# arkflow-rs/arkflow

Measured on AMD Instinct MI355X. Metric: rows/sec, higher is better.
Workload: dtype bf16; 1 GPU; model=generate→sql(filter)→mlp_anomaly[16→256→256→1], global_batch=8192, seq_len=1, parallelism=dp1, batch_size_per_gpu=8192, workers=1, filter=WHERE f0 >= 0.2

## Files before the change

### arkflow_amd/csrc/bindings.cpp

```cpp
#include <hip/hip_runtime.h>
#include <torch/extension.h>
#include <ATen/hip/HIPContext.h>

#include <algorithm>
#include <cstdint>
#include <limits>
#include <tuple>
#include <vector>

#include "gemm_api.h"
#include "kernels_api.h"
#include "relational_api.h"

namespace {

hipStream_t cur_stream() {
  return at::hip::getCurrentHIPStream().stream();
}

void check_cuda(const torch::Tensor& t, const char* name) {
  TORCH_CHECK(t.is_cuda(), name, " must be on GPU");
  TORCH_CHECK(t.is_contiguous(), name, " must be contiguous");
}

// ... 141 lines not shown
  TORCH_CHECK(keys.scalar_type() == torch::kInt64, "keys must be int64");
  int64_t n = keys.numel();
  auto opts32 = keys.options().dtype(torch::kInt32);
  if (n == 0)
    return {torch::empty({0}, opts32), torch::empty({0}, keys.options())};
  uint32_t tsize = next_pow2((uint32_t)std::max<int64_t>(n * 2, 64));
  auto table_keys = torch::empty({(int64_t)tsize}, keys.options());
  auto table_gids = torch::empty({(int64_t)tsize}, opts32);
  auto counter = torch::zeros({1}, opts32);
  auto gids = torch::empty({n}, opts32);
  auto st = cur_stream();
  launch_hash_build(keys.data_ptr<int64_t>(), n,
                    table_keys.data_ptr<int64_t>(),
                    table_gids.data_ptr<int32_t>(), tsize,
                    counter.data_ptr<int32_t>(), gids.data_ptr<int32_t>(), st);
  int64_t g = counter.item<int32_t>();
  auto uniq = torch::empty({g}, keys.options());
  launch_hash_export(table_keys.data_ptr<int64_t>(),
                     table_gids.data_ptr<int32_t>(), tsize,
                     uniq.data_ptr<int64_t>(), st);
  return {gids, uniq};
}

torch::Tensor segment_reduce_f32(torch::Tensor vals, torch::Tensor gids,
                                 int64_t g, int64_t op) {
  check_cuda(vals, "vals");
  check_cuda(gids, "gids");
  TORCH_CHECK(vals.scalar_type() == torch::kFloat32, "vals must be f32");
  auto g32 = gids.scalar_type() == torch::kInt32 ? gids
                                                 : gids.to(torch::kInt32);
  auto out = torch::zeros({g}, vals.options());
  if (vals.numel() == 0) return out;
  torch::Tensor scratch;
  int32_t* scratch_ptr = nullptr;
  if (op != 0) {
    scratch = torch::empty({g}, vals.options().dtype(torch::kInt32));
    scratch_ptr = scratch.data_ptr<int32_t>();
  }
  launch_segment_reduce_f32(vals.data_ptr<float>(), g32.data_ptr<int32_t>(),
                            vals.numel(), (int)g, (int)op,
                            out.data_ptr<float>(), scratch_ptr, cur_stream());
  return out;
}

std::tuple<torch::Tensor, torch::Tensor> join_inner_i64(torch::Tensor lk,
                                                        torch::Tensor rk) {
  check_cuda(lk, "left_keys");
  check_cuda(rk, "right_keys");
  TORCH_CHECK(lk.scalar_type() == torch::kInt64 &&
                  rk.scalar_type() == torch::kInt64,
              "join keys must be int64");
  int64_t nl = lk.numel(), nr = rk.numel();
  auto opts64 = lk.options();
  auto opts32 = lk.options().dtype(torch::kInt32);
  if (nl == 0 || nr == 0)
    return {torch::empty({0}, opts64), torch::empty({0}, opts64)};
  uint32_t tsize = next_pow2((uint32_t)std::max<int64_t>(nr * 2, 64));
  auto table_keys = torch::empty({(int64_t)tsize}, opts64);
  auto table_head = torch::empty({(int64_t)tsize}, opts32);
  auto next = torch::empty({nr}, opts32);
  auto st = cur_stream();
  launch_join_build(rk.data_ptr<int64_t>(), nr, table_keys.data_ptr<int64_t>(),
                    table_head.data_ptr<int32_t>(), next.data_ptr<int32_t>(),
                    tsize, st);
  auto counts = torch::empty({nl}, opts32);
  launch_join_probe_count(lk.data_ptr<int64_t>(), nl,
                          table_keys.data_ptr<int64_t>(),
                          table_head.data_ptr<int32_t>(),
                          next.data_ptr<int32_t>(), rk.data_ptr<int64_t>(),
                          tsize, counts.data_ptr<int32_t>(), st);
  auto [offs, total_t] = exscan(counts);
  int64_t total = total_t.item<int32_t>();
  auto l_out = torch::empty({total}, opts64);
  auto r_out = torch::empty({total}, opts64);
  if (total)
    launch_join_probe_emit(lk.data_ptr<int64_t>(), nl,
                           table_keys.data_ptr<int64_t>(),
                           table_head.data_ptr<int32_t>(),
                           next.data_ptr<int32_t>(), rk.data_ptr<int64_t>(),
                           tsize, offs.data_ptr<int32_t>(),
                           l_out.data_ptr<int64_t>(),
                           r_out.data_ptr<int64_t>(), st);
  return {l_out, r_out};
}

torch::Tensor device_vec_f32(const c10::optional<torch::Tensor>& v,
                             int64_t numel, const char* name) {
  if (!v.has_value() || !v->defined()) return torch::Tensor();
  TORCH_CHECK(v->is_cuda(), name, " must be on GPU");
  TORCH_CHECK(v->numel() == numel, name, " must have ", numel, " elements");
  return v->scalar_type() == torch::kFloat32
             ? v->contiguous()
             : v->to(torch::kFloat32).contiguous();
}

torch::Tensor check_gemm_args(const torch::Tensor& A, const torch::Tensor& Bt,
                              const c10::optional<torch::Tensor>& bias) {
  check_cuda(A, "A");
  check_cuda(Bt, "Bt");
  TORCH_CHECK(A.scalar_type() == torch::kBFloat16 &&
                  Bt.scalar_type() == torch::kBFloat16,
              "gemm_bf16 requires bf16 inputs");
  TORCH_CHECK(A.dim() == 2 && Bt.dim() == 2, "A [M,K], Bt [N,K]");
  int64_t K = A.size(1);
  TORCH_CHECK(Bt.size(1) == K, "K mismatch");
  TORCH_CHECK(K % 32 == 0 && K >= 32, "K must be a multiple of 32");
  return device_vec_f32(bias, Bt.size(0), "bias");
}

GemmArgs gemm_args(const torch::Tensor& A, const torch::Tensor& Bt,
                   const torch::Tensor& bias_f, torch::Tensor& C,
                   int64_t act) {
  return GemmArgs{A.data_ptr(), Bt.data_ptr(),
                  bias_f.defined() ? bias_f.data_ptr<float>() : nullptr,
                  C.data_ptr(), (int)A.size(0), (int)Bt.size(0),
                  (int)A.size(1), (int)act, cur_stream()};
}

torch::Tensor gemm_bf16(torch::Tensor A, torch::Tensor Bt,
                        c10::optional<torch::Tensor> bias, int64_t act) {
  auto bias_f = check_gemm_args(A, Bt, bias);
  int64_t M = A.size(0), K = A.size(1), N = Bt.size(0);
  auto C = torch::empty({M, N}, A.options());
  if (M == 0 || N == 0) return C;
  GemmArgs g = gemm_args(A, Bt, bias_f, C, act);
  int64_t t256 = ((M + 255) / 256) * ((N + 255) / 256);
  int rc = (t256 >= 128 && K >= 1536 && N >= 2048)
               ? launch_gemm_bf16(GEMM_8P256S, &g)
               : GEMM_BAD_SHAPE;
  if (rc != GEMM_OK) {
    int64_t t128grid = ((M + 127) / 128) * ((N + 127) / 128);
    if (t128grid < 208) {
      rc = launch_gemm_bf16(GEMM_SKINNY, &g);
    } else {
      rc = (K % 64 == 0) ? launch_gemm_bf16(GEMM_K64S, &g) : GEMM_BAD_SHAPE;
      if (rc != GEMM_OK) rc = launch_gemm_bf16(GEMM_BK32, &g);
    }
  }
  TORCH_CHECK(rc == GEMM_OK, "gemm_bf16: no kernel for this shape");
  return C;
}

torch::Tensor gemv_bf16_f32(torch::Tensor x, torch::Tensor w, double bias) {
  check_cuda(x, "x");
  check_cuda(w, "w");
  TORCH_CHECK(x.scalar_type() == torch::kBFloat16 &&
              w.scalar_type() == torch::kBFloat16, "bf16 required");
  TORCH_CHECK(x.dim() == 2 && w.numel() == x.size(1), "x [M,K], w [K]");
  auto out = torch::empty({x.size(0)}, x.options().dtype(torch::kFloat32));
  if (x.size(0) == 0) return out;
  launch_gemv_bf16_f32(x.data_ptr(), w.data_ptr(), (float)bias, x.size(0),
                       (int)x.size(1), out.data_ptr<float>(), cur_stream());
  return out;
}

void gen_fields(torch::Tensor block, c10::optional<torch::Tensor> key,
                std::vector<double> lo, std::vector<double> width,
                int64_t key_lo, int64_t key_range, torch::Tensor ctr) {
  check_cuda(block, "block");
  TORCH_CHECK(block.dim() == 2 && block.scalar_type() == torch::kFloat32,
              "block must be [nf, n] f32");
  TORCH_CHECK(ctr.scalar_type() == torch::kInt64 && ctr.numel() == 2,
              "ctr must be int64[2] on device");
  int nf = (int)block.size(0);
  int64_t n = block.size(1);
  TORCH_CHECK((int)lo.size() == nf && (int)width.size() == nf);
  std::vector<float> lof(nf), wf(nf);
  for (int f = 0; f < nf; ++f) { lof[f] = (float)lo[f]; wf[f] = (float)width[f]; }
  int64_t* key_ptr = nullptr;
  if (key.has_value() && key->defined()) {
    check_cuda(*key, "key");
    TORCH_CHECK(key->numel() == n && key->scalar_type() == torch::kInt64);
    key_ptr = key->data_ptr<int64_t>();
  } else {
    key_range = 0;
  }
  launch_gen_fields(block.data_ptr<float>(), key_ptr, n, lof.data(),
                    wf.data(), nf, key_lo, key_range,
                    (unsigned long long*)ctr.data_ptr<int64_t>(),
                    cur_stream());
}

void genfiltpack(std::vector<double> lo, std::vector<double> width,
                 int64_t key_lo, int64_t key_range, int64_t n, int64_t fidx,
                 int64_t op, double scalar,
                 std::vector<torch::Tensor> outs,
                 c10::optional<torch::Tensor> key_out,
                 c10::optional<torch::Tensor> feats,
                 torch::Tensor count_out, torch::Tensor counts_ws,
                 torch::Tensor bar, torch::Tensor ctr) {
  int nf = (int)outs.size();
  TORCH_CHECK(nf >= 1 && nf <= 32, "1..32 float columns");
  TORCH_CHECK((int)lo.size() == nf && (int)width.size() == nf);
  TORCH_CHECK(fidx >= 0 && fidx < nf, "fidx out of range");
  TORCH_CHECK(count_out.scalar_type() == torch::kInt32 &&
              count_out.numel() == 1);
  TORCH_CHECK(counts_ws.scalar_type() == torch::kInt32 &&
              counts_ws.numel() >= (n + 1023) / 1024);
  TORCH_CHECK(bar.scalar_type() == torch::kInt64 && bar.numel() >= 1);
  TORCH_CHECK(ctr.scalar_type() == torch::kInt64 && ctr.numel() == 2);
  std::vector<float> lof(nf), wf(nf);
  std::vector<float*> optr(nf);
  for (int f = 0; f < nf; ++f) {
    lof[f] = (float)lo[f];
    wf[f] = (float)width[f];
    check_cuda(outs[f], "out col");
    TORCH_CHECK(outs[f].numel() >= n &&
                outs[f].scalar_type() == torch::kFloat32);
    optr[f] = outs[f].data_ptr<float>();
  }
  int64_t* kptr = nullptr;
  if (key_out.has_value() && key_out->defined()) {
    TORCH_CHECK(key_out->numel() >= n &&
                key_out->scalar_type() == torch::kInt64);
    kptr = key_out->data_ptr<int64_t>();
  } else {
    key_range = 0;
  }
  void* fptr = nullptr;
  int dpad = 0;
  if (feats.has_value() && feats->defined()) {
    TORCH_CHECK(feats->dim() == 2 &&
                feats->scalar_type() == torch::kBFloat16 &&
                feats->size(0) >= n && feats->size(1) >= nf);
    fptr = feats->data_ptr();
    dpad = (int)feats->size(1);
  }
  int rc = launch_genfiltpack(
      lof.data(), wf.data(), nf, key_lo, key_range, n, (int)fidx, (int)op,
      (float)scalar, optr.data(), kptr, fptr, dpad,
      count_out.data_ptr<int32_t>(), counts_ws.data_ptr<int32_t>(),
      (unsigned long long*)bar.data_ptr<int64_t>(),
      (unsigned long long*)ctr.data_ptr<int64_t>(), cur_stream());
  TORCH_CHECK(rc == 0, "genfiltpack: batch too large for the in-kernel "
              "barrier (max 256K rows) — use the multi-kernel chain");
}

void featpack(std::vector<torch::Tensor> srcs, torch::Tensor out) {
  TORCH_CHECK(!srcs.empty() && srcs.size() <= 32, "1..32 feature columns");
  check_cuda(out, "out");
  TORCH_CHECK(out.dim() == 2 && out.scalar_type() == torch::kBFloat16,
              "out must be [n, kpad] bf16");
  int64_t n = out.size(0);
  int kpad = (int)out.size(1);
  TORCH_CHECK((int64_t)srcs.size() <= out.size(1),
              "out has fewer columns than sources");
  if (n == 0) return;
  bool f64 = srcs[0].scalar_type() == torch::kFloat64;
  if (f64) {
    std::vector<const double*> ptrs;
    for (auto& s : srcs) {
      check_cuda(s, "src");
      TORCH_CHECK(s.numel() >= n && s.scalar_type() == torch::kFloat64);
      ptrs.push_back(s.data_ptr<double>());
    }
    launch_featpack64(ptrs.data(), (int)ptrs.size(), kpad, n,
                      out.data_ptr(), cur_stream());
    return;
  }
  std::vector<const float*> ptrs;
  for (auto& s : srcs) {
    check_cuda(s, "src");
    TORCH_CHECK(s.numel() >= n && s.scalar_type() == torch::kFloat32);
    ptrs.push_back(s.data_ptr<float>());
  }
  launch_featpack(ptrs.data(), (int)ptrs.size(), kpad, n, out.data_ptr(),
                  cur_stream());
}

torch::Tensor gemm_bf16_variant(torch::Tensor A, torch::Tensor Bt,
                                c10::optional<torch::Tensor> bias,
                                int64_t act, int64_t variant) {
  auto bias_f = check_gemm_args(A, Bt, bias);
  auto C = torch::empty({A.size(0), Bt.size(0)}, A.options());
  if (C.numel() == 0) return C;
  GemmArgs g = gemm_args(A, Bt, bias_f, C, act);
  int rc = variant == (int)variant ? launch_gemm_bf16((int)variant, &g)
                                   : (int)GEMM_BAD_VARIANT;
  TORCH_CHECK(rc != GEMM_BAD_VARIANT, "unknown gemm variant ", variant);
  TORCH_CHECK(rc == GEMM_OK, "K = ", g.K,
              " not supported by gemm variant ", variant);
  return C;
}

torch::Tensor layernorm_bf16(torch::Tensor x, torch::Tensor gamma,
                             torch::Tensor beta, double eps,
                             c10::optional<torch::Tensor> residual) {
  check_cuda(x, "x");
  TORCH_CHECK(x.scalar_type() == torch::kBFloat16, "x must be bf16");
  TORCH_CHECK(x.dim() >= 1 && x.size(-1) > 0, "x must be [..., n], n > 0");
  int64_t n = x.size(-1);
  TORCH_CHECK(n % 8 == 0, "inner dim must be a multiple of 8");
  int64_t rows = x.numel() / n;
  TORCH_CHECK(gamma.defined() && beta.defined(), "gamma and beta required");
  auto g = device_vec_f32(gamma, n, "gamma");
  auto b = device_vec_f32(beta, n, "beta");
  auto out = torch::empty_like(x);
  const void* res_ptr = nullptr;
  if (residual.has_value() && residual->defined()) {
    check_cuda(*residual, "residual");
    TORCH_CHECK(residual->scalar_type() == torch::kBFloat16,
                "residual must be bf16");
    TORCH_CHECK(residual->sizes() == x.sizes(),
                "residual must have x's shape");
    res_ptr = residual->data_ptr();
  }
// ... 591 lines not shown
void check_rows(const torch::Tensor& t, const char* name,
                torch::ScalarType ty, int64_t n) {
  check_cuda(t, name);
  TORCH_CHECK(t.scalar_type() == ty, name, " has the wrong dtype");
  TORCH_CHECK(t.dim() == 1 && t.numel() == n, name, " must have one entry ",
              "per row");
}

torch::Tensor segmented_scan(torch::Tensor vals, torch::Tensor head,
                             int64_t op, bool reverse) {
  int64_t n = vals.numel();
  TORCH_CHECK(n < (int64_t(1) << 31), "row indices are int32");
  TORCH_CHECK(op >= SCAN_SUM && op <= SCAN_MAX, "unknown scan op ", op);
  check_rows(vals, "values", torch::kFloat64, n);
  check_rows(head, "head", torch::kUInt8, n);
  return seg_scan(vals, head, (int)op, reverse);
}

std::tuple<torch::Tensor, torch::Tensor> window_frame(
    torch::Tensor vals, c10::optional<torch::Tensor> valid,
    torch::Tensor part, c10::optional<int64_t> lo, c10::optional<int64_t> hi,
    int64_t func, c10::optional<torch::Tensor> perm) {
  int64_t n = part.numel();
  TORCH_CHECK(n < (int64_t(1) << 31), "row indices are int32");
  TORCH_CHECK(func >= WF_SUM && func <= WF_COUNT_STAR,
              "unknown window function ", func);
  TORCH_CHECK(!lo || !hi || *lo <= *hi, "frame start is after frame end");
  check_rows(part, "partition ids", torch::kInt64, n);
  check_rows(vals, "values", torch::kFloat64, n);
  if (valid) check_rows(*valid, "validity", torch::kUInt8, n);
  if (perm) check_rows(*perm, "perm", torch::kInt64, n);
  auto f64 = vals.options();
  auto u8 = vals.options().dtype(torch::kUInt8);
  auto out = torch::empty({n}, f64);
  auto out_valid = torch::empty({n}, u8);
  if (n == 0) return {out, out_valid};
  auto st = cur_stream();
  if (lo) lo = std::max(-n, std::min(n, *lo));
  if (hi) hi = std::max(-n, std::min(n, *hi));

  auto head = torch::empty({n}, u8), tail = torch::empty({n}, u8);
  auto head_idx = torch::empty({n}, f64), tail_idx = torch::empty({n}, f64);
  launch_win_bounds(part.data_ptr<int64_t>(), n, head.data_ptr<uint8_t>(),
                    tail.data_ptr<uint8_t>(), head_idx.data_ptr<double>(),
                    tail_idx.data_ptr<double>(), st);
  auto start = seg_scan(head_idx, head, SCAN_MAX, false);
  auto end = seg_scan(tail_idx, tail, SCAN_MIN, true);

  const bool is_sum = func == WF_SUM || func == WF_AVG;
  const bool is_minmax = func == WF_MIN || func == WF_MAX;
  const bool sliding = is_minmax && lo && hi;
  const bool need_count = valid && (is_sum || is_minmax || func == WF_COUNT);
  const int64_t width = sliding ? *hi - *lo + 1 : 1;
  const double inf = std::numeric_limits<double>::infinity();
  const double fill = func == WF_MIN ? inf : func == WF_MAX ? -inf : 0.0;

  torch::Tensor masked, ones, chunk_head, chunk_tail, prefix, suffix, count;
  if (is_sum || is_minmax) masked = torch::empty({n}, f64);
  if (need_count) ones = torch::empty({n}, f64);
  if (sliding) {
    chunk_head = torch::empty({n}, u8);
    chunk_tail = torch::empty({n}, u8);
  }
  auto ptr_f64 = [](const torch::Tensor& t) {
    return t.defined() ? t.data_ptr<double>() : nullptr;
  };
  auto ptr_u8 = [](const torch::Tensor& t) {
    return t.defined() ? t.data_ptr<uint8_t>() : nullptr;
  };
  const uint8_t* valid_p = valid ? valid->data_ptr<uint8_t>() : nullptr;
  if (masked.defined() || ones.defined())
    launch_win_inputs(vals.data_ptr<double>(), valid_p,
                      start.data_ptr<double>(), end.data_ptr<double>(), n,
                      fill, width, ptr_f64(masked), ptr_f64(ones),
                      ptr_u8(chunk_head), ptr_u8(chunk_tail), st);
  if (need_count) count = seg_scan(ones, head, SCAN_SUM, false);
  if (is_sum) prefix = seg_scan(masked, head, SCAN_SUM, false);
  if (is_minmax) {
    const int op = func == WF_MIN ? SCAN_MIN : SCAN_MAX;
    if (sliding || !lo)
      prefix = seg_scan(masked, sliding ? chunk_head : head, op, false);
    if (sliding || lo)
      suffix = seg_scan(masked, sliding ? chunk_tail : tail, op, true);
  }

  FrameArgs a{};
  a.start = start.data_ptr<double>();
  a.end = end.data_ptr<double>();
  a.vals = vals.data_ptr<double>();
  a.valid = valid_p;
  a.prefix = ptr_f64(prefix);
  a.suffix = ptr_f64(suffix);
  a.count = ptr_f64(count);
  a.perm = perm ? perm->data_ptr<int64_t>() : nullptr;
  a.lo = lo.value_or(0);
  a.hi = hi.value_or(0);
  a.lo_unbounded = !lo;
  a.hi_unbounded = !hi;
  a.func = (int)func;
  a.n = n;
  a.out = out.data_ptr<double>();
  a.out_valid = out_valid.data_ptr<uint8_t>();
  launch_win_frame(&a, st);
  return {out, out_valid};
}

}

PYBIND11_MODULE(TORCH_EXTENSION_NAME, m) {
  m.doc() = "arkflow_amd gfx950 native kernels";
  m.def("exclusive_offsets", &exclusive_offsets);
  m.def("take_binary", &take_binary);
  m.def("bytes_match", &bytes_match);
  m.def("attention_qkv_bf16", &attention_qkv_bf16, py::arg("qkv"),
        py::arg("scale"), py::arg("pad") = 8, py::arg("lens") = py::none());
  m.def("mask_to_indices", &mask_to_indices);
  m.def("filter_cmp_scalar", &filter_cmp_scalar);
  m.def("gather", &gather);
  m.def("hash_group_i64", &hash_group_i64);
  m.def("segment_reduce_f32", &segment_reduce_f32);
  m.def("join_inner_i64", &join_inner_i64);
  m.def("gemm_bf16", &gemm_bf16, py::arg("A"), py::arg("Bt"),
        py::arg("bias") = py::none(), py::arg("act") = 0);
  m.def("layernorm_bf16", &layernorm_bf16, py::arg("x"), py::arg("gamma"),
        py::arg("beta"), py::arg("eps") = 1e-5,
        py::arg("residual") = py::none());
  m.def("softmax_bf16", &softmax_bf16, py::arg("x"), py::arg("scale") = 1.0);
  m.def("mapped_int32", &mapped_int32, py::arg("n"));
  m.def("bias_act_bf16", &bias_act_bf16, py::arg("x"),
        py::arg("bias") = py::none(), py::arg("act") = 0);
  m.def("attention_bf16", &attention_bf16, py::arg("q"), py::arg("k"),
        py::arg("v"), py::arg("scale"), py::arg("lens") = py::none());
  m.def("proto_decode", &proto_decode, py::arg("data"),
        py::arg("offsets"), py::arg("fno"), py::arg("kind"),
        py::arg("is_float"), py::arg("slot"), py::arg("n_int"),
        py::arg("n_float"), py::arg("n_str"), py::arg("capture") = false);
  m.def("gather_columns", &gather_columns);
  m.def("gemm_bf16_variant", &gemm_bf16_variant);
  m.def("bytes_hash", &bytes_hash);
  m.def("json_decode", &json_decode);
  m.def("fused_filter_gather", &fused_filter_gather);
  m.def("genfiltpack", &genfiltpack, py::arg("lo"), py::arg("width"),
        py::arg("key_lo"), py::arg("key_range"), py::arg("n"),
        py::arg("fidx"), py::arg("op"), py::arg("scalar"), py::arg("outs"),
        py::arg("key_out"), py::arg("feats"), py::arg("count_out"),
        py::arg("counts_ws"), py::arg("bar"), py::arg("ctr"));
  m.def("fused_filter_agg", &fused_filter_agg);
  m.def("hash_agg_capture", &hash_agg_capture, py::arg("keys"),
        py::arg("nrow"), py::arg("vals"), py::arg("ops"),
        py::arg("table_size"), py::arg("g_cap"),
        py::arg("gcount_out") = c10::nullopt);
  m.def("filter_gather_capture", &filter_gather_capture);
  m.def("gemv_bf16_f32", &gemv_bf16_f32);
  m.def("gen_fields", &gen_fields);
  m.def("featpack", &featpack);
  m.def("radix_argsort", &radix_argsort, py::arg("keys"), py::arg("descending") = false);
  m.def("segmented_scan", &segmented_scan, py::arg("values"), py::arg("head"),
        py::arg("op"), py::arg("reverse") = false);
  m.def("seg_scan_tile_rows", &seg_scan_tile_rows);
  m.def("window_frame", &window_frame, py::arg("values"), py::arg("valid"),
        py::arg("part"), py::arg("lo"), py::arg("hi"), py::arg("func"),
        py::arg("perm") = py::none());
}
```

### arkflow_amd/csrc/gemm_api.h

```cpp
#pragma once
#include <hip/hip_runtime.h>

enum GemmVariant {
  GEMM_BK32 = 0,
  GEMM_8P256 = 1,
  GEMM_8P256S = 2,
  GEMM_2P = 3,
  GEMM_8P128 = 4,
  GEMM_8P128S = 5,
  GEMM_SKINNY = 6,
  GEMM_K64 = 7,
  GEMM_K64S = 8,
  GEMM_K64D = 9,
  GEMM_K64P = 10,
  GEMM_K64W = 11,
  GEMM_K64S3 = 12,
};

enum GemmStatus {
  GEMM_OK = 0,
  GEMM_BAD_SHAPE = 1,
  GEMM_BAD_VARIANT = 2,
};

struct GemmArgs {
  const void* A;
  const void* Bt;
  const float* bias;
  void* C;
  int M, N, K;
  int act;
  hipStream_t stream;
};

extern "C" int launch_gemm_bf16(int variant, const GemmArgs* args);
```

### arkflow_amd/csrc/gemm_common.h

```cpp
#pragma once
#include <hip/hip_runtime.h>

#include <type_traits>

#include "common.h"
#include "gemm_api.h"

typedef __attribute__((ext_vector_type(8))) __bf16 bf16x8;
typedef __attribute__((ext_vector_type(4))) float f32x4;
typedef __attribute__((ext_vector_type(4))) uint32_t u32x4;

enum Act { ACT_NONE = 0, ACT_RELU = 1, ACT_GELU = 2, ACT_SILU = 3 };

DEV_INLINE float apply_act(float x, int act) {
  switch (act) {
    case ACT_RELU: return fmaxf(x, 0.f);
    case ACT_GELU: {
      float c = 0.7978845608028654f * (x + 0.044715f * x * x * x);
      c = fminf(fmaxf(c, -10.f), 10.f);
      float e = __expf(2.f * c);
      return 0.5f * x * (1.f + (e - 1.f) / (e + 1.f));
    }
    case ACT_SILU: return x / (1.f + __expf(-x));
    default: return x;
  }
}

DEV_INLINE int xcd_block_id() {
  int nwg = gridDim.x;
  int bid = blockIdx.x;
  if (nwg >= 16) {
    int q = nwg / 8, r = nwg % 8;
    int xcd = bid % 8, off = bid / 8;
    bid = (xcd < r ? xcd * (q + 1) : r * (q + 1) + (xcd - r) * q) + off;
  }
  return bid;
}


template <int TILE, int BKT, int THREADS>
DEV_INLINE void stage_direct(const __bf16* __restrict__ A,
                             const __bf16* __restrict__ Bt, int row0, int col0,
                             int M, int N, int K, int k0, __bf16* Asm,
                             __bf16* Bsm) {
  constexpr int ROW_BYTES = BKT * 2;
  constexpr int STEPS = TILE * ROW_BYTES / (THREADS * 16);
  const int lane = threadIdx.x & 63;
  const int wid = threadIdx.x >> 6;
#pragma unroll
  for (int it = 0; it < STEPS; ++it) {
    int wbase = wid * 1024 + it * THREADS * 16;
    int lin = wbase + lane * 16;
    int trow = lin / ROW_BYTES;
    int tcol = lin % ROW_BYTES;
    int ga_row = min(row0 + trow, M - 1);
    const char* a_src = (const char*)(A + (int64_t)ga_row * K + k0) + tcol;
    __builtin_amdgcn_global_load_lds(
        (const __attribute__((address_space(1))) uint32_t*)a_src,
        (__attribute__((address_space(3))) uint32_t*)((char*)Asm + wbase),
        16, 0, 0);
    int gb_row = min(col0 + trow, N - 1);
    const char* b_src = (const char*)(Bt + (int64_t)gb_row * K + k0) + tcol;
    __builtin_amdgcn_global_load_lds(
        (const __attribute__((address_space(1))) uint32_t*)b_src,
        (__attribute__((address_space(3))) uint32_t*)((char*)Bsm + wbase),
        16, 0, 0);
  }
}

constexpr int SWZ_BK = 64;
constexpr int SWZ_STEPS = 4;

template <int TILE>
DEV_INLINE void swz_load(const __bf16* __restrict__ A,
                         const __bf16* __restrict__ Bt, int row0, int col0,
                         int M, int N, int K, int k0, u32x4 (&va)[SWZ_STEPS],
                         u32x4 (&vb)[SWZ_STEPS]) {
  const int lin0 = (threadIdx.x >> 6) * 1024 + (threadIdx.x & 63) * 16;
#pragma unroll
  for (int it = 0; it < SWZ_STEPS; ++it) {
    int lin = lin0 + it * (2 * TILE * 16);
    int trow = lin >> 7;
    int tcol = lin & 127;
    int ga_row = min(row0 + trow, M - 1);
    va[it] = *(const u32x4*)((const char*)(A + (int64_t)ga_row * K + k0) +
                             tcol);
    int gb_row = min(col0 + trow, N - 1);
    vb[it] = *(const u32x4*)((const char*)(Bt + (int64_t)gb_row * K + k0) +
                             tcol);
  }
}

template <int TILE>
DEV_INLINE void swz_write(__bf16* Asm, __bf16* Bsm,
                          const u32x4 (&va)[SWZ_STEPS],
                          const u32x4 (&vb)[SWZ_STEPS]) {
  const int lin0 = (threadIdx.x >> 6) * 1024 + (threadIdx.x & 63) * 16;
#pragma unroll
  for (int it = 0; it < SWZ_STEPS; ++it) {
    int lin = lin0 + it * (2 * TILE * 16);
    int trow = lin >> 7;
    int tcol = lin & 127;
    int dst = (trow << 7) + (((tcol >> 4) ^ (trow & 7)) << 4);
    *(u32x4*)((char*)Asm + dst) = va[it];
    *(u32x4*)((char*)Bsm + dst) = vb[it];
  }
}

template <int FM, int FN, int BKT, bool SWZ>
DEV_INLINE void load_frags(const __bf16* Asm, const __bf16* Bsm, int wm,
                           int wn, int ks, bf16x8 (&a_frag)[FM],
                           bf16x8 (&b_frag)[FN]) {
  const int lane = threadIdx.x & 63;
  const int fr = lane & 15;
  const int chunk = ks * 4 + (lane >> 4);
#pragma unroll
  for (int m = 0; m < FM; ++m) {
    int row = wm + m * 16 + fr;
    a_frag[m] =
        *(const bf16x8*)&Asm[row * BKT + (SWZ ? chunk ^ (row & 7) : chunk) * 8];
  }
#pragma unroll
  for (int n = 0; n < FN; ++n) {
    int row = wn + n * 16 + fr;
    b_frag[n] =
        *(const bf16x8*)&Bsm[row * BKT + (SWZ ? chunk ^ (row & 7) : chunk) * 8];
  }
}

template <int FM, int FN>
DEV_INLINE void mma_frags(const bf16x8 (&a_frag)[FM],
                          const bf16x8 (&b_frag)[FN], f32x4 (&acc)[FM][FN]) {
#pragma unroll
  for (int m = 0; m < FM; ++m)
#pragma unroll
    for (int n = 0; n < FN; ++n)
      acc[m][n] = __builtin_amdgcn_mfma_f32_16x16x32_bf16(
          a_frag[m], b_frag[n], acc[m][n], 0, 0, 0);
}

template <int FM, int FN, int BKT, bool SWZ>
DEV_INLINE void mma_slice(const __bf16* Asm, const __bf16* Bsm, int wm, int wn,
                          f32x4 (&acc)[FM][FN]) {
#pragma unroll
  for (int ks = 0; ks < BKT / 32; ++ks) {
    bf16x8 a_frag[FM], b_frag[FN];
    load_frags<FM, FN, BKT, SWZ>(Asm, Bsm, wm, wn, ks, a_frag, b_frag);
    mma_frags<FM, FN>(a_frag, b_frag, acc);
  }
}

template <int ACT, bool HAS_BIAS, int FM, int FN, class RowOf, class ColOf>
DEV_INLINE void store_frags(const f32x4 (&acc)[FM][FN],
                            const float* __restrict__ bias,
                            __bf16* __restrict__ C, int M, int N,
                            RowOf frag_row, ColOf frag_col) {
  const int lane = threadIdx.x & 63;
#pragma unroll
  for (int m = 0; m < FM; ++m) {
#pragma unroll
    for (int n = 0; n < FN; ++n) {
      int col = frag_col(n) + (lane & 15);
      if (col >= N) continue;
      float b = HAS_BIAS ? bias[col] : 0.f;
#pragma unroll
      for (int r = 0; r < 4; ++r) {
        int row = frag_row(m) + (lane >> 4) * 4 + r;
        if (row >= M) continue;
        C[(int64_t)row * N + col] = (__bf16)apply_act(acc[m][n][r] + b, ACT);
      }
    }
  }
}

template <int ACT, bool HAS_BIAS, int FM, int FN>
DEV_INLINE void store_tile(const f32x4 (&acc)[FM][FN],
                           const float* __restrict__ bias,
                           __bf16* __restrict__ C, int M, int N, int wrow,
                           int wcol) {
  store_frags<ACT, HAS_BIAS>(
      acc, bias, C, M, N, [&](int m) { return wrow + m * 16; },
      [&](int n) { return wcol + n * 16; });
}

template <class F>
static void dispatch_epilogue(int act, bool has_bias, F&& f) {
  auto with_act = [&](auto a) {
    if (has_bias) f(a, std::true_type{});
    else f(a, std::false_type{});
  };
  switch (act) {
    case ACT_RELU: with_act(std::integral_constant<int, ACT_RELU>{}); break;
    case ACT_GELU: with_act(std::integral_constant<int, ACT_GELU>{}); break;
    case ACT_SILU: with_act(std::integral_constant<int, ACT_SILU>{}); break;
    default: with_act(std::integral_constant<int, ACT_NONE>{}); break;
  }
}

template <int BMT, int BNT, class Kernel>
static void launch_tiles(Kernel kernel, int threads, size_t lds_bytes,
                         const GemmArgs& g) {
  int tiles_n = cdiv(g.N, BNT);
  hipLaunchKernelGGL(kernel, dim3(cdiv(g.M, BMT) * tiles_n), dim3(threads),
                     lds_bytes, g.stream, (const __bf16*)g.A,
                     (const __bf16*)g.Bt, g.bias, (__bf16*)g.C, g.M, g.N, g.K,
                     tiles_n);
}

int launch_gemm_bf16_8p(const GemmArgs& g, int bm, bool swz);
```

### arkflow_amd/csrc/stepfused.hip

```cpp
#include "common.h"
#include "kernels_api.h"

DEV_INLINE float u01(uint64_t h) {
  return (float)(h >> 40) * (1.0f / 16777216.0f);
}

struct GenSpec {
  float lo[32];
  float width[32];
  int nf;
  int64_t key_lo;
  int64_t key_range;
};

__global__ void gen_fields_kernel(float* __restrict__ block,
                                  int64_t* __restrict__ key, int64_t n,
                                  GenSpec spec,
                                  unsigned long long* __restrict__ ctr) {
  uint64_t c = ctr[0];
  int64_t i = (int64_t)blockIdx.x * blockDim.x + threadIdx.x;
  int64_t stride = (int64_t)gridDim.x * blockDim.x;
  for (; i < n; i += stride) {
    uint64_t base = (c << 32) ^ (uint64_t)i;
#pragma unroll 4
    for (int f = 0; f < spec.nf; ++f) {
      uint64_t h = mix64(base + ((uint64_t)(f + 1) << 52));
      block[(int64_t)f * n + i] = spec.lo[f] + spec.width[f] * u01(h);
    }
    if (spec.key_range > 0) {
      uint64_t h = mix64(base + (0x9E37ull << 48));
      key[i] = spec.key_lo + (int64_t)(h % (uint64_t)spec.key_range);
    }
  }
  __syncthreads();
  if (threadIdx.x == 0) {
    unsigned long long t = atomicAdd(&ctr[1], 1ull);
    if (t == (unsigned long long)gridDim.x - 1) {
      ctr[1] = 0ull;
      ctr[0] = c + 1ull;
      __threadfence();
    }
  }
}

extern "C" void launch_gen_fields(float* block, int64_t* key, int64_t n,
                                  const float* lo, const float* width,
                                  int nf, int64_t key_lo, int64_t key_range,
                                  unsigned long long* ctr, hipStream_t st) {
  GenSpec spec{};
  spec.nf = nf > 32 ? 32 : nf;
  for (int f = 0; f < spec.nf; ++f) {
    spec.lo[f] = lo[f];
    spec.width[f] = width[f];
  }
  spec.key_lo = key_lo;
  spec.key_range = key_range;
  int grid = (int)((n + 255) / 256);
  if (grid > 1024) grid = 1024;
  if (grid < 1) return;
  gen_fields_kernel<<<grid, 256, 0, st>>>(block, key, n, spec, ctr);
}

__global__ void scan_counts_kernel(const int32_t* __restrict__ counts, int nb,
                                   int32_t* __restrict__ offs,
                                   int32_t* __restrict__ total) {
  __shared__ int32_t lds[1024];
  int tid = threadIdx.x;
  int v = tid < nb ? counts[tid] : 0;
  lds[tid] = v;
  __syncthreads();
  for (int s = 1; s < 1024; s <<= 1) {
    int add = tid >= s ? lds[tid - s] : 0;
    __syncthreads();
    lds[tid] += add;
    __syncthreads();
  }
  if (tid < nb) offs[tid] = lds[tid] - v;
  if (tid == nb - 1) *total = lds[tid];
}

extern "C" void launch_scan_counts(const int32_t* counts, int nb,
                                   int32_t* offs, int32_t* total,
                                   hipStream_t st) {
  scan_counts_kernel<<<1, 1024, 0, st>>>(counts, nb, offs, total);
}

struct GfpOuts {
  float* outs[32];
  int64_t* key_out;
  __bf16* feats;
  int32_t* count_out;
  int32_t* counts_ws;
  unsigned long long* bar;
  unsigned long long* ctr;
};

#define GFP_CH 1024

__global__ __launch_bounds__(256)
void genfiltpack_kernel(GenSpec spec, int64_t n, int ch, int fidx, int op,
                        float scalar, int dpad, GfpOuts o) {
  const uint64_t c = o.ctr[0];
  const int b = blockIdx.x, grid = gridDim.x;
  const int tid = threadIdx.x;
  const int lane = tid & 63, wid = tid >> 6;
  const int64_t start = (int64_t)b * ch;
  __shared__ uint16_t loc[GFP_CH];
  __shared__ int wave_base[5];
  __shared__ int lcount_sh;
  __shared__ int base_sh;
  if (tid == 0) lcount_sh = 0;
  __syncthreads();
  for (int s = 0; s < ch / 256; ++s) {
    int64_t idx = start + s * 256 + tid;
    bool pred = false;
    if (idx < n) {
      uint64_t rb = (c << 32) ^ (uint64_t)idx;
      uint64_t h = mix64(rb + ((uint64_t)(fidx + 1) << 52));
      float v = spec.lo[fidx] + spec.width[fidx] * u01(h);
      switch (op) {
        case 0: pred = v < scalar; break;
        case 1: pred = v <= scalar; break;
        case 2: pred = v > scalar; break;
        case 3: pred = v >= scalar; break;
        case 4: pred = v == scalar; break;
        default: pred = v != scalar; break;
      }
    }
    uint64_t ballot = __ballot(pred);
    int rank = __popcll(ballot & lanemask_lt());
    if (lane == 0) wave_base[wid + 1] = __popcll(ballot);
    __syncthreads();
    if (tid == 0) {
      wave_base[0] = lcount_sh;
      for (int w = 1; w <= 4; ++w) wave_base[w] += wave_base[w - 1];
      lcount_sh = wave_base[4];
    }
    __syncthreads();
    if (pred) loc[wave_base[wid] + rank] = (uint16_t)(s * 256 + tid);
    __syncthreads();
  }
  const int lcount = lcount_sh;
  if (tid == 0)
    __hip_atomic_store(&o.counts_ws[b], lcount, __ATOMIC_RELEASE,
                       __HIP_MEMORY_SCOPE_AGENT);
  if (tid == 0) {
    unsigned long long old = atomicAdd(o.bar, 1ull);
    unsigned long long target =
        (old / grid + 1) * (unsigned long long)grid;
    while (__hip_atomic_load(o.bar, __ATOMIC_ACQUIRE,
                             __HIP_MEMORY_SCOPE_AGENT) < target)
      __builtin_amdgcn_s_sleep(8);
  }
  __syncthreads();
  if (tid == 0) {
    int basev = 0, total = 0;
    for (int j = 0; j < grid; ++j) {
      int v = __hip_atomic_load(&o.counts_ws[j], __ATOMIC_RELAXED,
                                __HIP_MEMORY_SCOPE_AGENT);
      if (j < b) basev += v;
      total += v;
    }
    base_sh = basev;
    if (b == 0) *o.count_out = total;
  }
  __syncthreads();
  const int base_out = base_sh;
  for (int j = tid; j < lcount; j += 256) {
    int64_t r = start + loc[j];
    int64_t dst = base_out + j;
    uint64_t rb = (c << 32) ^ (uint64_t)r;
    for (int f = 0; f < spec.nf; ++f) {
      uint64_t h = mix64(rb + ((uint64_t)(f + 1) << 52));
      float v = spec.lo[f] + spec.width[f] * u01(h);
      o.outs[f][dst] = v;
      if (o.feats) o.feats[dst * dpad + f] = (__bf16)v;
    }
    if (spec.key_range > 0) {
      uint64_t h = mix64(rb + (0x9E37ull << 48));
      o.key_out[dst] =
          spec.key_lo + (int64_t)(h % (uint64_t)spec.key_range);
    }
  }
  __syncthreads();
  if (tid == 0) {
    unsigned long long t = atomicAdd(&o.ctr[1], 1ull);
    if (t == (unsigned long long)grid - 1) {
      o.ctr[1] = 0ull;
      o.ctr[0] = c + 1ull;
      __threadfence();
    }
  }
}

extern "C" int launch_genfiltpack(const float* lo, const float* width,
                                  int nf, int64_t key_lo, int64_t key_range,
                                  int64_t n, int fidx, int op, float scalar,
                                  float* const* outs, int64_t* key_out,
                                  void* feats, int dpad, int32_t* count_out,
                                  int32_t* counts_ws,
                                  unsigned long long* bar,
                                  unsigned long long* ctr, hipStream_t st) {
  int ch = GFP_CH;
  while (ch > 256 && (n + ch - 1) / ch < 64) ch >>= 1;
  int grid = (int)((n + ch - 1) / ch);
  if (grid < 1 || grid > 256 || nf > 32) return -1;
  GenSpec spec{};
  spec.nf = nf;
  for (int f = 0; f < nf; ++f) {
    spec.lo[f] = lo[f];
    spec.width[f] = width[f];
  }
  spec.key_lo = key_lo;
  spec.key_range = key_range;
  GfpOuts o{};
  for (int f = 0; f < nf; ++f) o.outs[f] = outs[f];
  o.key_out = key_out;
  o.feats = (__bf16*)feats;
  o.count_out = count_out;
  o.counts_ws = counts_ws;
  o.bar = bar;
  o.ctr = ctr;
  genfiltpack_kernel<<<grid, 256, 0, st>>>(spec, n, ch, fidx, op, scalar,
                                           dpad, o);
  return 0;
}

struct PackSpec {
  const float* src[32];
  int nf;
  int kpad;
};

__global__ void featpack_kernel(PackSpec spec, int64_t n,
                                __bf16* __restrict__ out) {
  int64_t i = (int64_t)blockIdx.x * blockDim.x + threadIdx.x;
  int64_t stride = (int64_t)gridDim.x * blockDim.x;
  for (; i < n; i += stride) {
    __bf16* row = out + i * spec.kpad;
#pragma unroll 4
    for (int f = 0; f < spec.nf; ++f) row[f] = (__bf16)spec.src[f][i];
    for (int f = spec.nf; f < spec.kpad; ++f) row[f] = (__bf16)0.f;
  }
}

extern "C" void launch_featpack(const float** src, int nf, int kpad,
                                int64_t n, void* out, hipStream_t st) {
  PackSpec spec{};
  spec.nf = nf > 32 ? 32 : nf;
  spec.kpad = kpad;
  for (int f = 0; f < spec.nf; ++f) spec.src[f] = src[f];
  int grid = (int)((n + 255) / 256);
  if (grid > 2048) grid = 2048;
  if (grid < 1) return;
  featpack_kernel<<<grid, 256, 0, st>>>(spec, n, (__bf16*)out);
}

struct PackSpec64 {
  const double* src[32];
  int nf;
  int kpad;
};

__global__ void featpack64_kernel(PackSpec64 spec, int64_t n,
                                  __bf16* __restrict__ out) {
  int64_t i = (int64_t)blockIdx.x * blockDim.x + threadIdx.x;
  int64_t stride = (int64_t)gridDim.x * blockDim.x;
  for (; i < n; i += stride) {
    __bf16* row = out + i * spec.kpad;
#pragma unroll 4
    for (int f = 0; f < spec.nf; ++f) {
      float v = (float)spec.src[f][i];
      asm volatile("" : "+v"(v));
      row[f] = (__bf16)v;
    }
    for (int f = spec.nf; f < spec.kpad; ++f) row[f] = (__bf16)0.f;
  }
}

extern "C" void launch_featpack64(const double** src, int nf, int kpad,
                                  int64_t n, void* out, hipStream_t st) {
  PackSpec64 spec{};
  spec.nf = nf > 32 ? 32 : nf;
  spec.kpad = kpad;
  for (int f = 0; f < spec.nf; ++f) spec.src[f] = src[f];
  int grid = (int)((n + 255) / 256);
  if (grid > 2048) grid = 2048;
  if (grid < 1) return;
  featpack64_kernel<<<grid, 256, 0, st>>>(spec, n, (__bf16*)out);
}

__global__ void gemv_bf16_f32_kernel(const __bf16* __restrict__ x,
                                     const __bf16* __restrict__ w,
                                     float bias, int64_t M, int K,
                                     float* __restrict__ out) {
  int64_t wave = ((int64_t)blockIdx.x * blockDim.x + threadIdx.x) >> 6;
  int lane = threadIdx.x & 63;
  int64_t row0 = wave * 8;
  if (row0 >= M) return;
  int sub = lane >> 3;
  int piece = lane & 7;
  int64_t row = row0 + sub;
  if (row >= M) return;
  const __bf16* xr = x + row * K;
  float acc = 0.f;
  for (int k = piece; k < K; k += 8) acc += (float)xr[k] * (float)w[k];
  for (int off = 1; off < 8; off <<= 1) {
    float o = __shfl_down(acc, off, 64);
    if (piece + off < 8) acc += o;
  }
  if (piece == 0) out[row] = acc + bias;
}

extern "C" void launch_gemv_bf16_f32(const void* x, const void* w, float bias,
                                     int64_t M, int K, float* out,
                                     hipStream_t st) {
  int64_t waves = (M + 7) / 8;
  int64_t threads = waves * 64;
  int grid = (int)((threads + 255) / 256);
  if (grid < 1) return;
  gemv_bf16_f32_kernel<<<grid, 256, 0, st>>>((const __bf16*)x,
                                             (const __bf16*)w, bias, M, K,
                                             out);
}
```

### arkflow_amd/models/mlp.py

```python
from __future__ import annotations

from typing import List, Sequence

import torch

from ..ops import nn as opsnn


class MlpAnomalyDetector:
    def __init__(self, in_features: int, hidden: Sequence[int] = (256, 256),
                 device: torch.device = torch.device("cpu"), seed: int = 1234):
        self.device = torch.device(device)
        self.in_features = in_features
        gen = torch.Generator().manual_seed(seed)
        dims = [_pad32(in_features), *[_pad32(h) for h in hidden], 1]
        self.weights: List[torch.Tensor] = []
        self.biases: List[torch.Tensor] = []
        for i in range(len(dims) - 1):
            k = dims[i]
            n = dims[i + 1]
            w = torch.randn(n, k, generator=gen) * (k ** -0.5)
            b = torch.randn(n, generator=gen) * 0.01
            self.weights.append(w.to(self.device, torch.bfloat16))
            self.biases.append(b.to(self.device, torch.float32))
        self.dims = dims
        self.use_graph = True
        self._graphs = {}
        self._head_bias = None

    def forward(self, x: torch.Tensor) -> torch.Tensor:
        if self.use_graph and self.device.type == "cuda":
            return self._forward_graphed(x)
        return self._forward_eager(x)

    def _forward_eager(self, x: torch.Tensor) -> torch.Tensor:
        h = x.to(self.device, torch.bfloat16)
        pad = _pad32(self.in_features) - self.in_features
        if pad:
            h = torch.nn.functional.pad(h, (0, pad))
        return self._net(h)

    def _net(self, h: torch.Tensor) -> torch.Tensor:
        for i, (w, b) in enumerate(zip(self.weights, self.biases)):
            last = i == len(self.weights) - 1
            if last and h.is_cuda and w.shape[0] == 1:
                from ..ops import require_native
                if self._head_bias is None:
                    self._head_bias = float(b[0].item())
                return require_native().gemv_bf16_f32(
                    h.contiguous(), w.reshape(-1).contiguous(),
                    self._head_bias)
            act = "relu" if not last else "none"
            h = opsnn.linear_bf16(h, w, b, act=act)
        return h.reshape(-1).to(torch.float32)

    def _forward_graphed(self, x: torch.Tensor) -> torch.Tensor:
        n = x.shape[0]
        cap = self._cap_for(n)
        entry = self._graphs.get(cap)
        if entry is None:
            static_in = torch.zeros(cap, _pad32(self.in_features),
                                    device=self.device, dtype=torch.bfloat16)
            s = torch.cuda.Stream()
            s.wait_stream(torch.cuda.current_stream())
            with torch.cuda.stream(s):
                for _ in range(2):
                    self._net(static_in)
            torch.cuda.current_stream().wait_stream(s)
            graph = torch.cuda.CUDAGraph()
            with torch.cuda.graph(graph, capture_error_mode="thread_local"):
                static_out = self._net(static_in)
            entry = (graph, static_in, static_out)
            self._graphs[cap] = entry
        graph, static_in, static_out = entry
        static_in[:n, : self.in_features].copy_(
            x.to(self.device, torch.bfloat16))
        graph.replay()
        return static_out[:n].clone()

    @staticmethod
    def _cap_for(n: int) -> int:
        cap = 4096
        while cap < n:
            cap <<= 1
        return cap


def _pad32(k: int) -> int:
    return (k + 31) // 32 * 32
```

### setup.py

```python
import os

from setuptools import Extension, setup

os.environ.setdefault("PYTORCH_ROCM_ARCH", "gfx950")

from torch.utils.cpp_extension import BuildExtension, CUDAExtension

ROOT = os.path.dirname(os.path.abspath(__file__))
CSRC = os.path.join(ROOT, "arkflow_amd", "csrc")

sources = [
    os.path.join(CSRC, f)
    for f in ("bindings.cpp", "filter.hip", "hash_agg.hip", "hash_join.hip",
              "gemm_bf16.hip", "gemm_8phase.hip", "rowops.hip", "attention.hip", "proto_decode.hip", "radix_sort.hip", "json_decode.hip",
              "stepfused.hip", "window.hip")
]

setup(
    name="arkflow_amd_native",
    ext_modules=[
        CUDAExtension(
            name="arkflow_amd._native",
            sources=sources,
            extra_compile_args={
                "cxx": ["-O3", "-std=c++17"],
                "nvcc": ["-O3", "-std=c++17"],
            },
        ),
        Extension(
            name="arkflow_amd._wal_native",
            sources=[os.path.join(CSRC, "wal_codec.cpp")],
            extra_compile_args=["-O3", "-std=c++17"],
        ),
    ],
    cmdclass={"build_ext": BuildExtension.with_options(use_ninja=True)},
)
```

Before: 156.0 million rows/s.

## Add fused three-layer MLP kernel and vectorize genfiltpack feature writes

Adds a single HIP kernel that runs the 16→256→256→1 MLP per 32-row tile. Layer-1 activations stay in LDS and layer-2 weights in registers, which removes intermediate global traffic and separate launches; this path is enabled only through an environment flag. The generate/filter/pack kernel now reduces per-block counts with a wave-level parallel reduction instead of one serial thread. It also writes packed bf16 feature rows as 16-byte vectors. The fused kernel holds many registers per thread, which may reduce occupancy.

```diff
diff --git a/arkflow_amd/csrc/bindings.cpp b/arkflow_amd/csrc/bindings.cpp
--- a/arkflow_amd/csrc/bindings.cpp
+++ b/arkflow_amd/csrc/bindings.cpp
@@ -317,6 +317,53 @@
   launch_gemv_bf16_f32(x.data_ptr(), w.data_ptr(), (float)bias, x.size(0),
                        (int)x.size(1), out.data_ptr<float>(), cur_stream());
   return out;
+}
+
+torch::Tensor mlp3_bf16_f32(torch::Tensor x, torch::Tensor w1, torch::Tensor b1,
+                            torch::Tensor w2, torch::Tensor b2,
+                            torch::Tensor w3, double bias3,
+                            c10::optional<torch::Tensor> out) {
+  check_cuda(x, "x");
+  check_cuda(w1, "w1");
+  check_cuda(w2, "w2");
+  check_cuda(w3, "w3");
+  TORCH_CHECK(x.scalar_type() == torch::kBFloat16 &&
+                  w1.scalar_type() == torch::kBFloat16 &&
+                  w2.scalar_type() == torch::kBFloat16 &&
+                  w3.scalar_type() == torch::kBFloat16,
+              "mlp3_bf16_f32 requires bf16 x, w1, w2, w3");
+  TORCH_CHECK(x.dim() == 2 && w1.dim() == 2 && w2.dim() == 2,
+              "x [M,K0], w1 [H1,K0], w2 [H2,H1]");
+  int64_t M = x.size(0), K0 = x.size(1), H1 = w1.size(0), H2 = w2.size(0);
+  TORCH_CHECK(w1.size(1) == K0, "w1 must be [H1,K0]");
+  TORCH_CHECK(w2.size(1) == H1, "w2 must be [H2,H1]");
+  TORCH_CHECK(w3.numel() == H2, "w3 must have H2 elements");
+  TORCH_CHECK(M < (int64_t)std::numeric_limits<int32_t>::max() - 256,
+              "too many rows");
+  auto b1f = device_vec_f32(b1, H1, "b1");
+  auto b2f = device_vec_f32(b2, H2, "b2");
+  for (const torch::Tensor* t : {&x, &w1, &w2})
+    TORCH_CHECK((uintptr_t)t->data_ptr() % 16 == 0,
+                "x, w1, w2 must be 16-byte aligned");
+  torch::Tensor scores;
+  if (out.has_value() && out->defined()) {
+    scores = *out;
+    check_cuda(scores, "out");
+    TORCH_CHECK(scores.scalar_type() == torch::kFloat32 &&
+                    scores.dim() == 1 && scores.size(0) == M,
+                "out must be f32 [M]");
+  } else {
+    scores = torch::empty({M}, x.options().dtype(torch::kFloat32));
+  }
+  Mlp3Args a{x.data_ptr(),  w1.data_ptr(),          b1f.data_ptr<float>(),
+             w2.data_ptr(), b2f.data_ptr<float>(),  w3.data_ptr(),
+             (float)bias3,  scores.data_ptr<float>(), (int)M,
+             (int)K0,       (int)H1,                (int)H2,
+             cur_stream()};
+  int rc = launch_mlp3_bf16_f32(&a);
+  TORCH_CHECK(rc == GEMM_OK, "mlp3_bf16_f32: K0 must be a multiple of 32 in "
+              "[32, 256] and H1, H2 each 64, 128 or 256");
+  return scores;
 }
 
 void gen_fields(torch::Tensor block, c10::optional<torch::Tensor> key,
@@ -1214,6 +1261,10 @@
         py::arg("gcount_out") = c10::nullopt);
   m.def("filter_gather_capture", &filter_gather_capture);
   m.def("gemv_bf16_f32", &gemv_bf16_f32);
+  m.def("mlp3_bf16_f32", &mlp3_bf16_f32, py::arg("x"), py::arg("w1"),
+        py::arg("b1"), py::arg("w2"), py::arg("b2"), py::arg("w3"),
+        py::arg("bias3"), py::arg("out") = c10::nullopt);
+  m.attr("MLP3_BM") = MLP3_BM;
   m.def("gen_fields", &gen_fields);
   m.def("featpack", &featpack);
   m.def("radix_argsort", &radix_argsort, py::arg("keys"), py::arg("descending") = false);
diff --git a/arkflow_amd/csrc/gemm_api.h b/arkflow_amd/csrc/gemm_api.h
--- a/arkflow_amd/csrc/gemm_api.h
+++ b/arkflow_amd/csrc/gemm_api.h
@@ -34,3 +34,20 @@
 };
 
 extern "C" int launch_gemm_bf16(int variant, const GemmArgs* args);
+
+struct Mlp3Args {
+  const void* X;
+  const void* W1;
+  const float* b1;
+  const void* W2;
+  const float* b2;
+  const void* w3;
+  float bias3;
+  float* out;
+  int M, K0, H1, H2;
+  hipStream_t stream;
+};
+
+constexpr int MLP3_BM = 32;
+
+extern "C" int launch_mlp3_bf16_f32(const Mlp3Args* args);
diff --git a/arkflow_amd/csrc/gemm_common.h b/arkflow_amd/csrc/gemm_common.h
--- a/arkflow_amd/csrc/gemm_common.h
+++ b/arkflow_amd/csrc/gemm_common.h
@@ -68,6 +68,32 @@
   }
 }
 
+template <int ROWS, int BKT, int THREADS>
+DEV_INLINE void stage_direct_one(const __bf16* __restrict__ S, int row0,
+                                 int nrows, int K, int k0, __bf16* sm) {
+  constexpr int ROW_BYTES = BKT * 2;
+  constexpr int BYTES = ROWS * ROW_BYTES;
+  constexpr int STEP_BYTES = THREADS * 16;
+  static_assert(BYTES % 1024 == 0, "a wave stages whole 1 KiB pieces");
+  constexpr int STEPS = (BYTES + STEP_BYTES - 1) / STEP_BYTES;
+  const int lane = threadIdx.x & 63;
+  const int wid = threadIdx.x >> 6;
+#pragma unroll
+  for (int it = 0; it < STEPS; ++it) {
+    int wbase = wid * 1024 + it * STEP_BYTES;
+    if (BYTES % STEP_BYTES != 0 && wbase >= BYTES) break;
+    int lin = wbase + lane * 16;
+    int trow = lin / ROW_BYTES;
+    int tcol = lin % ROW_BYTES;
+    int g_row = min(row0 + trow, nrows - 1);
+    const char* src = (const char*)(S + (int64_t)g_row * K + k0) + tcol;
+    __builtin_amdgcn_global_load_lds(
+        (const __attribute__((address_space(1))) uint32_t*)src,
+        (__attribute__((address_space(3))) uint32_t*)((char*)sm + wbase),
+        16, 0, 0);
+  }
+}
+
 constexpr int SWZ_BK = 64;
 constexpr int SWZ_STEPS = 4;
 
@@ -125,6 +151,18 @@
     int row = wn + n * 16 + fr;
     b_frag[n] =
         *(const bf16x8*)&Bsm[row * BKT + (SWZ ? chunk ^ (row & 7) : chunk) * 8];
+  }
+}
+
+template <int FM>
+DEV_INLINE void load_a_frags_strided(const __bf16* Asm, int stride, int wm,
+                                     int kofs, bf16x8 (&a_frag)[FM]) {
+  const int lane = threadIdx.x & 63;
+  const int fr = lane & 15;
+#pragma unroll
+  for (int m = 0; m < FM; ++m) {
+    int row = wm + m * 16 + fr;
+    a_frag[m] = *(const bf16x8*)&Asm[row * stride + kofs + (lane >> 4) * 8];
   }
 }
 
diff --git a/arkflow_amd/csrc/mlp_fused.hip b/arkflow_amd/csrc/mlp_fused.hip
--- /dev/null
+++ b/arkflow_amd/csrc/mlp_fused.hip
@@ -0,0 +1,139 @@
+#include "gemm_common.h"
+
+#define MLP3_THREADS 256
+
+template <int FM, int FN>
+DEV_INLINE void relu_frags_to_lds(const f32x4 (&acc)[FM][FN],
+                                  const float (&bias)[FN], __bf16* Hs,
+                                  int stride, int wn) {
+  const int lane = threadIdx.x & 63;
+#pragma unroll
+  for (int m = 0; m < FM; ++m) {
+#pragma unroll
+    for (int n = 0; n < FN; ++n) {
+      int col = wn + n * 16 + (lane & 15);
+#pragma unroll
+      for (int r = 0; r < 4; ++r) {
+        int row = m * 16 + (lane >> 4) * 4 + r;
+        Hs[row * stride + col] =
+            (__bf16)apply_act(acc[m][n][r] + bias[n], ACT_RELU);
+      }
+    }
+  }
+}
+
+template <int BM, int H1, int H2>
+__global__ __launch_bounds__(MLP3_THREADS)
+void mlp3_kernel(const __bf16* __restrict__ X,
+                 const __bf16* __restrict__ W1,
+                 const float* __restrict__ b1,
+                 const __bf16* __restrict__ W2,
+                 const float* __restrict__ b2,
+                 const __bf16* __restrict__ w3,
+                 float bias3, float* __restrict__ out, int M, int K0) {
+  constexpr int FM = BM / 16;
+  constexpr int FN1 = H1 / 64, FN2 = H2 / 64;
+  constexpr int KS2 = H1 / 32;
+  constexpr int S1 = H1 + 8, S2 = H2 + 8;
+  constexpr int SMAX = S1 > S2 ? S1 : S2;
+  __shared__ alignas(16) __bf16 Xs[BM * 32];
+  __shared__ alignas(16) __bf16 Ws[H1 * 32];
+  __shared__ alignas(16) __bf16 Hs[BM * SMAX];
+  __shared__ __bf16 w3s[H2];
+
+  const int tid = threadIdx.x;
+  const int lane = tid & 63;
+  const int wid = tid >> 6;
+  const int row0 = blockIdx.x * BM;
+  const int wn1 = wid * (FN1 * 16);
+  const int wn2 = wid * (FN2 * 16);
+
+  if (tid < H2) w3s[tid] = w3[tid];
+  float bias1[FN1], bias2[FN2];
+#pragma unroll
+  for (int n = 0; n < FN1; ++n) bias1[n] = b1[wn1 + n * 16 + (lane & 15)];
+#pragma unroll
+  for (int n = 0; n < FN2; ++n) bias2[n] = b2[wn2 + n * 16 + (lane & 15)];
+  bf16x8 w2f[KS2][FN2];
+#pragma unroll
+  for (int ks = 0; ks < KS2; ++ks)
+#pragma unroll
+    for (int n = 0; n < FN2; ++n)
+      w2f[ks][n] = *(const bf16x8*)&W2[(wn2 + n * 16 + (lane & 15)) * H1 +
+                                       ks * 32 + (lane >> 4) * 8];
+
+  f32x4 acc1[FM][FN1] = {};
+  for (int k0 = 0; k0 < K0; k0 += 32) {
+    stage_direct_one<BM, 32, MLP3_THREADS>(X, row0, M, K0, k0, Xs);
+    stage_direct_one<H1, 32, MLP3_THREADS>(W1, 0, H1, K0, k0, Ws);
+    __syncthreads();
+    bf16x8 a_frag[FM], b_frag[FN1];
+    load_frags<FM, FN1, 32, false>(Xs, Ws, 0, wn1, 0, a_frag, b_frag);
+    mma_frags<FM, FN1>(a_frag, b_frag, acc1);
+    __syncthreads();
+  }
+  relu_frags_to_lds<FM, FN1>(acc1, bias1, Hs, S1, wn1);
+  __syncthreads();
+
+  f32x4 acc2[FM][FN2] = {};
+#pragma unroll
+  for (int ks = 0; ks < KS2; ++ks) {
+    bf16x8 a_frag[FM];
+    load_a_frags_strided<FM>(Hs, S1, 0, ks * 32, a_frag);
+    mma_frags<FM, FN2>(a_frag, w2f[ks], acc2);
+  }
+  __syncthreads();
+  relu_frags_to_lds<FM, FN2>(acc2, bias2, Hs, S2, wn2);
+  __syncthreads();
+
+  constexpr int LPR = MLP3_THREADS / BM;
+  constexpr int PP = 8 / LPR;
+  const int hrow = tid / LPR;
+  const int q = tid % LPR;
+  const __bf16* hr = Hs + hrow * S2;
+  float part[PP] = {};
+  for (int k = 0; k < H2; k += 8) {
+#pragma unroll
+    for (int i = 0; i < PP; ++i) {
+      int kk = k + q * PP + i;
+      part[i] += (float)hr[kk] * (float)w3s[kk];
+    }
+  }
+  float acc = part[0];
+  if (PP == 2) acc += part[PP - 1];
+#pragma unroll
+  for (int off = 1; off < LPR; off <<= 1) acc += __shfl_down(acc, off, 64);
+  if (q == 0 && row0 + hrow < M) out[row0 + hrow] = acc + bias3;
+}
+
+template <int BM, int H1, int H2>
+static void launch_mlp3(const Mlp3Args& a) {
+  hipLaunchKernelGGL((mlp3_kernel<BM, H1, H2>), dim3(cdiv(a.M, BM)),
+                     dim3(MLP3_THREADS), 0, a.stream, (const __bf16*)a.X,
+                     (const __bf16*)a.W1, a.b1, (const __bf16*)a.W2, a.b2,
+                     (const __bf16*)a.w3, a.bias3, a.out, a.M, a.K0);
+}
+
+template <class F>
+static bool with_hidden(int h, F&& f) {
+  switch (h) {
+    case 64: f(std::integral_constant<int, 64>{}); return true;
+    case 128: f(std::integral_constant<int, 128>{}); return true;
+    case 256: f(std::integral_constant<int, 256>{}); return true;
+    default: return false;
+  }
+}
+
+extern "C" int launch_mlp3_bf16_f32(const Mlp3Args* args) {
+  const Mlp3Args& a = *args;
+  if (a.K0 < 32 || a.K0 > 256 || a.K0 % 32 != 0) return GEMM_BAD_SHAPE;
+  auto ok = [](int h) { return h == 64 || h == 128 || h == 256; };
+  if (!ok(a.H1) || !ok(a.H2)) return GEMM_BAD_SHAPE;
+  if (a.M <= 0) return GEMM_OK;
+  with_hidden(a.H1, [&](auto h1) {
+    with_hidden(a.H2, [&](auto h2) {
+      launch_mlp3<MLP3_BM, decltype(h1)::value, decltype(h2)::value>(a);
+    });
+  });
+  return GEMM_OK;
+}
diff --git a/arkflow_amd/csrc/stepfused.hip b/arkflow_amd/csrc/stepfused.hip
--- a/arkflow_amd/csrc/stepfused.hip
+++ b/arkflow_amd/csrc/stepfused.hip
@@ -94,6 +94,8 @@
   unsigned long long* bar;
   unsigned long long* ctr;
 };
+
+typedef __attribute__((ext_vector_type(8))) __bf16 gfp_bf16x8;
 
 #define GFP_CH 1024
 
@@ -153,28 +155,50 @@
       __builtin_amdgcn_s_sleep(8);
   }
   __syncthreads();
-  if (tid == 0) {
+  if (wid == 0) {
     int basev = 0, total = 0;
-    for (int j = 0; j < grid; ++j) {
+    for (int j = lane; j < grid; j += 64) {
       int v = __hip_atomic_load(&o.counts_ws[j], __ATOMIC_RELAXED,
                                 __HIP_MEMORY_SCOPE_AGENT);
       if (j < b) basev += v;
       total += v;
     }
-    base_sh = basev;
-    if (b == 0) *o.count_out = total;
+    for (int off = 32; off > 0; off >>= 1) {
+      basev += __shfl_down(basev, off, 64);
+      total += __shfl_down(total, off, 64);
+    }
+    if (lane == 0) {
+      base_sh = basev;
+      if (b == 0) *o.count_out = total;
+    }
   }
   __syncthreads();
   const int base_out = base_sh;
+  const bool feats16 =
+      o.feats && dpad % 8 == 0 && ((uintptr_t)o.feats & 15) == 0;
   for (int j = tid; j < lcount; j += 256) {
     int64_t r = start + loc[j];
     int64_t dst = base_out + j;
     uint64_t rb = (c << 32) ^ (uint64_t)r;
-    for (int f = 0; f < spec.nf; ++f) {
-      uint64_t h = mix64(rb + ((uint64_t)(f + 1) << 52));
-      float v = spec.lo[f] + spec.width[f] * u01(h);
-      o.outs[f][dst] = v;
-      if (o.feats) o.feats[dst * dpad + f] = (__bf16)v;
+    for (int f0 = 0; f0 < spec.nf; f0 += 8) {
+      const int nv = min(8, spec.nf - f0);
+      gfp_bf16x8 pk = {};
+#pragma unroll
+      for (int i = 0; i < 8; ++i) {
+        if (i >= nv) break;
+        int f = f0 + i;
+        uint64_t h = mix64(rb + ((uint64_t)(f + 1) << 52));
+        float v = spec.lo[f] + spec.width[f] * u01(h);
+        o.outs[f][dst] = v;
+        pk[i] = (__bf16)v;
+      }
+      if (!o.feats) continue;
+      __bf16* frow = o.feats + dst * dpad + f0;
+      if (feats16 && nv == 8) {
+        *(gfp_bf16x8*)frow = pk;
+      } else {
+        for (int i = 0; i < nv; ++i) frow[i] = pk[i];
+      }
     }
     if (spec.key_range > 0) {
       uint64_t h = mix64(rb + (0x9E37ull << 48));
diff --git a/arkflow_amd/models/mlp.py b/arkflow_amd/models/mlp.py
--- a/arkflow_amd/models/mlp.py
+++ b/arkflow_amd/models/mlp.py
@@ -1,5 +1,6 @@
 from __future__ import annotations
 
+import os
 from typing import List, Sequence
 
 import torch
@@ -40,7 +41,21 @@
             h = torch.nn.functional.pad(h, (0, pad))
         return self._net(h)
 
+    def _fusable(self) -> bool:
+        d = self.dims
+        return (len(d) == 4 and d[3] == 1 and d[0] <= 256
+                and d[1] in _MLP3_HIDDEN and d[2] in _MLP3_HIDDEN)
+
     def _net(self, h: torch.Tensor) -> torch.Tensor:
+        if (h.is_cuda and self._fusable()
+                and os.environ.get("ARKFLOW_MLP_FUSED", "0") == "1"):
+            from ..ops import require_native
+            if self._head_bias is None:
+                self._head_bias = float(self.biases[2][0].item())
+            w1, w2, w3 = self.weights
+            return require_native().mlp3_bf16_f32(
+                h.contiguous(), w1, self.biases[0], w2, self.biases[1],
+                w3.reshape(-1), self._head_bias)
         for i, (w, b) in enumerate(zip(self.weights, self.biases)):
             last = i == len(self.weights) - 1
             if last and h.is_cuda and w.shape[0] == 1:
@@ -86,5 +101,8 @@
         return cap
 
 
+_MLP3_HIDDEN = (64, 128, 256)
+
+
 def _pad32(k: int) -> int:
     return (k + 31) // 32 * 32
diff --git a/setup.py b/setup.py
--- a/setup.py
+++ b/setup.py
@@ -13,7 +13,7 @@
     os.path.join(CSRC, f)
     for f in ("bindings.cpp", "filter.hip", "hash_agg.hip", "hash_join.hip",
               "gemm_bf16.hip", "gemm_8phase.hip", "rowops.hip", "attention.hip", "proto_decode.hip", "radix_sort.hip", "json_decode.hip",
-              "stepfused.hip", "window.hip")
+              "stepfused.hip", "window.hip", "mlp_fused.hip")
 ]
 
 setup(
```

Result: no change. 154.9 million rows/s (-0.8%).
